# pixeru/bpm_analysis

Hardware: AMD Instinct MI355X
Metric: audio-samples/sec (filter+envelope+peaks), 1024x60s@44.1kHz batch, 1 & 8 GPU (higher is better)
Workload: dtype f64; 1 GPU; 1024 x 60 s 44100 Hz mono int16 recordings per GPU, native mode (filter+envelope+noise floor+raw peaks); mode=native, parallelism=file-sharded x1, batch_pipeline=False

## Files before the change

bpm_analysis_amd/csrc/k_envelope_native.hip:

```cpp
#include <rocfft/rocfft.h>

#include <algorithm>
#include <cstring>
#include <cstdlib>
#include <map>
#include <mutex>
#include <tuple>
#include <vector>

#include <complex>

#include "bpmx_common.h"
#include "bpmx_kernels.h"
#include "bpmx_native.h"
#include "bpmx_hilbert.h"
#ifndef BPMX_NM_POLICY
#define BPMX_NM_POLICY " nt"
#endif
#include "bpmx_qsel.h"
#include "bpmx_xlane.h"

namespace bpmx {

enum { TB_A = 0, TB_V = 0, TB_B = 16, TB_C = 20, TB_D = 24, TB_M = 25, TB_P = 41, TB_ZI = 57, TB_COEF = 64 };

enum { TT_KPOW = 0, TT_MT = 96, TT_G0 = 112, TT_ALPHA = 128, TT_BETA = 384, TT_VI = 640, TT_SIZE = 656 };
constexpr int NAT_PART = 16;
constexpr int NAT_DSMAX = 1280;

struct NatTile {
    int64_t s0;
    int64_t gbase;
    int64_t ybase;
    int32_t j0, nb;
    int32_t f, pad;
};

__device__ __forceinline__ NatTile nat_tile_ld(const NatTile *p, int64_t t) {
    typedef const __attribute__((address_space(4))) int64_t c64;
    c64 *q = (c64 *)(p + __builtin_amdgcn_readfirstlane((int)t));
    NatTile r;
    r.s0 = q[0]; r.gbase = q[1]; r.ybase = q[2];
    const int64_t a = q[3], b = q[4];
    r.j0 = (int32_t)a; r.nb = (int32_t)(a >> 32); r.f = (int32_t)b; r.pad = (int32_t)(b >> 32);
    return r;
}

struct NatBlockArgs {
    const void *pcm;
    const NatTile *tiles;
    int64_t n_tiles, total;
    int32_t bt, channels, ds;
    const double *tab, *tt;
    double *gam;
    double *agg;
    double *part;
};

struct NatCarryArgs {
    const void *pcm;
    const int64_t *foff, *doff, *boff, *toff;
    const int32_t *active;
    int32_t n_files, dtype, channels, ds, bt;
    const double *tab, *tt, *agg;
    double *part;
    double *carry;
    double *yd;
    InitOutArgs io;
    const double *ttab;
};
constexpr int NAT_TT_ROWS = NAT_DSMAX + 20, NAT_TT_PAR = 320;

struct NatYdArgs {
    const NatTile *tiles;
    const int32_t *skip;
    int32_t bt;
    const double *tt, *carry, *gam;
    double *yd;
};

struct NatEnvArgs {
    const double *y;
    const double *h;
    const int64_t *doff;
    const int32_t *active;
    int32_t n_files, window;
    double *env;
    const int32_t *skip;
};

struct V4 { double a, b, c, d; };
struct M4 { double m[16]; };

__device__ __forceinline__ V4 mv(const M4 &M, const V4 &x) {
    V4 r;
    r.a = __builtin_fma(M.m[0], x.a, __builtin_fma(M.m[1], x.b, __builtin_fma(M.m[2], x.c, M.m[3] * x.d)));
    r.b = __builtin_fma(M.m[4], x.a, __builtin_fma(M.m[5], x.b, __builtin_fma(M.m[6], x.c, M.m[7] * x.d)));
    r.c = __builtin_fma(M.m[8], x.a, __builtin_fma(M.m[9], x.b, __builtin_fma(M.m[10], x.c, M.m[11] * x.d)));
    r.d = __builtin_fma(M.m[12], x.a, __builtin_fma(M.m[13], x.b, __builtin_fma(M.m[14], x.c, M.m[15] * x.d)));
    return r;
}
__device__ __forceinline__ V4 mv_rot(const double *r, const V4 &x) {
    const double a1 = r[0], b1 = r[1], a2 = r[2], b2 = r[3];
    return V4{__builtin_fma(a1, x.a, b1 * x.b), __builtin_fma(a1, x.b, -b1 * x.a), __builtin_fma(a2, x.c, b2 * x.d),
              __builtin_fma(a2, x.d, -b2 * x.c)};
}
__device__ __forceinline__ V4 add4(const V4 &x, const V4 &y) { return V4{x.a + y.a, x.b + y.b, x.c + y.c, x.d + y.d}; }
__device__ __forceinline__ V4 acc_rot(const V4 &acc, const double *r, const V4 &x) {
    const double a1 = r[0], b1 = r[1], a2 = r[2], b2 = r[3];
    return V4{__builtin_fma(a1, x.a, __builtin_fma(b1, x.b, acc.a)), __builtin_fma(a1, x.b, __builtin_fma(-b1, x.a, acc.b)),
              __builtin_fma(a2, x.c, __builtin_fma(b2, x.d, acc.c)), __builtin_fma(a2, x.d, __builtin_fma(-b2, x.c, acc.d))};
}
__device__ __forceinline__ M4 mm(const M4 &X, const M4 &Y) {
    M4 R;
#pragma unroll
    for (int i = 0; i < 4; ++i)
#pragma unroll
        for (int j = 0; j < 4; ++j)
            R.m[i * 4 + j] = __builtin_fma(X.m[i * 4 + 0], Y.m[0 * 4 + j],
                             __builtin_fma(X.m[i * 4 + 1], Y.m[1 * 4 + j],
                             __builtin_fma(X.m[i * 4 + 2], Y.m[2 * 4 + j], X.m[i * 4 + 3] * Y.m[3 * 4 + j])));
    return R;
}
__device__ __forceinline__ M4 eye4() {
    M4 R;
#pragma unroll
    for (int i = 0; i < 16; ++i) R.m[i] = (i % 5 == 0) ? 1.0 : 0.0;
    return R;
}
__device__ __forceinline__ M4 shfl_up_m(const M4 &X, int d) {
    M4 R;
#pragma unroll
    for (int i = 0; i < 16; ++i) R.m[i] = __shfl_up(X.m[i], d);
    return R;
}
__device__ __forceinline__ M4 shfl_down_m(const M4 &X, int d) {
    M4 R;
#pragma unroll
    for (int i = 0; i < 16; ++i) R.m[i] = __shfl_down(X.m[i], d);
    return R;
}
__device__ __forceinline__ V4 shfl_v(const V4 &x, int src) {
    return V4{__shfl(x.a, src), __shfl(x.b, src), __shfl(x.c, src), __shfl(x.d, src)};
}
__device__ __forceinline__ V4 shfl_up_v(const V4 &x, int d) {
    return V4{__shfl_up(x.a, d), __shfl_up(x.b, d), __shfl_up(x.c, d), __shfl_up(x.d, d)};
}
__device__ __forceinline__ V4 shfl_down_v(const V4 &x, int d) {
    return V4{__shfl_down(x.a, d), __shfl_down(x.b, d), __shfl_down(x.c, d), __shfl_down(x.d, d)};
}
template <int D>
__device__ __forceinline__ V4 xl_up_v(const V4 &x) {
    return V4{xl_up<D>(x.a), xl_up<D>(x.b), xl_up<D>(x.c), xl_up<D>(x.d)};
}
template <int D>
__device__ __forceinline__ V4 xl_down_v(const V4 &x) {
    return V4{xl_down<D>(x.a), xl_down<D>(x.b), xl_down<D>(x.c), xl_down<D>(x.d)};
}
__device__ __forceinline__ M4 mpow(const M4 &X, int64_t e) {
    M4 R = eye4(), P = X;
    while (e > 0) {
        if (e & 1) R = mm(P, R);
        P = mm(P, P);
        e >>= 1;
    }
    return R;
}

struct SosStep {
    double s[12];
    __device__ __forceinline__ double step(V4 &z, double u) const {
        const double x1 = s[0] * u + z.a;
        const double z00 = s[1] * u - s[4] * x1 + z.b;
        const double z01 = s[2] * u - s[5] * x1;
        const double y = s[6] * x1 + z.c;
        const double z10 = s[7] * x1 - s[10] * y + z.d;
        const double z11 = s[8] * x1 - s[11] * y;
        z = V4{z00, z01, z10, z11};
        return y;
    }
};


template <int DT, bool MULTI>
__device__ __forceinline__ double nat_frame(const void *__restrict__ pcm, int ch, int64_t frame) {
    if (!MULTI) {
        switch (DT) {
        case BPMX_DT_U8: return (double)((const uint8_t *)pcm)[frame];
        case BPMX_DT_I16: return (double)((const int16_t *)pcm)[frame];
        case BPMX_DT_I32: return (double)((const int32_t *)pcm)[frame];
        case BPMX_DT_F32: return (double)((const float *)pcm)[frame];
        default: return ((const double *)pcm)[frame];
        }
    }
    return frame_value(pcm, DT, ch, frame);
}

__device__ __forceinline__ V4 nat_ld4(const double *p) { return V4{p[0], p[1], p[2], p[3]}; }
__device__ __forceinline__ M4 nat_ld16(const double *p) {
    M4 r;
#pragma unroll
    for (int i = 0; i < 16; ++i) r.m[i] = p[i];
    return r;
}
__device__ __forceinline__ double dot4(const V4 &a, const V4 &b) {
    return __builtin_fma(a.a, b.a, __builtin_fma(a.b, b.b, __builtin_fma(a.c, b.c, a.d * b.d)));
}

enum { ET_KPOW = 0, ET_P = 24, ET_C = 40, ET_D = 44, ET_SIZE = 45 };
__device__ __forceinline__ void nat_stage_epilogue_tables(const NatBlockArgs &A, double *et) {
    for (int i = threadIdx.x; i < ET_SIZE; i += blockDim.x) {
        double v;
        if (i < ET_P) v = A.tt[TT_KPOW + i];
        else if (i < ET_C) v = A.tab[TB_P + i - ET_P];
        else if (i < ET_D) v = A.tab[TB_C + i - ET_C];
        else v = A.tab[TB_D];
        et[i] = v;
    }
}

__device__ __forceinline__ void nat_tile_epilogue(const NatBlockArgs &A, const double *et, const NatTile &tl,
                                                  int64_t t, int lane, bool valid, V4 u, V4 v, double x) {
    const int bt = A.bt;
    const int Lt = tl.nb - tl.j0 < bt ? tl.nb - tl.j0 : bt;
    if (Lt < bt) {
        if (valid) {
            double *pp = A.part + ((int64_t)tl.f * 64 + lane) * NAT_PART;
            pp[0] = u.a; pp[1] = u.b; pp[2] = u.c; pp[3] = u.d;
            pp[4] = v.a; pp[5] = v.b; pp[6] = v.c; pp[7] = v.d;
            pp[8] = x;
        }
        return;
    }
    if (!valid) { u = V4{0, 0, 0, 0}; v = V4{0, 0, 0, 0}; x = 0; }
    V4 incl = u;
#define NAT_UP(K)                                                            \
    {                                                                        \
        const V4 y = K == 0 ? xl_up_v<1>(incl) : shfl_up_v(incl, 1 << K);   \
        if (lane >= (1 << K)) incl = acc_rot(incl, et + ET_KPOW + 4 * K, y);   \
    }
    NAT_UP(0) NAT_UP(1) NAT_UP(2) NAT_UP(3) NAT_UP(4) NAT_UP(5)
#undef NAT_UP
    V4 loc = xl_up_v<1>(incl);
    if (lane == 0) loc = V4{0, 0, 0, 0};
    V4 R = valid ? add4(mv(nat_ld16(et + ET_P), loc), v) : V4{0, 0, 0, 0};
#define NAT_DOWN(K)                                                          \
    {                                                                        \
        const V4 y = K == 0 ? xl_down_v<1>(R) : shfl_down_v(R, 1 << K);      \
        if (lane + (1 << K) < 64) R = acc_rot(R, et + ET_KPOW + 4 * K, y);     \
    }
    NAT_DOWN(0) NAT_DOWN(1) NAT_DOWN(2) NAT_DOWN(3) NAT_DOWN(4) NAT_DOWN(5)
#undef NAT_DOWN
    const V4 C = nat_ld4(et + ET_C);
    const double D = et[ET_D];
    if (valid) A.gam[tl.gbase + lane] = dot4(C, R) + D * dot4(C, loc) + D * D * x;
    double *ag = A.agg + t * 8;
    if (lane == bt - 1) { ag[0] = incl.a; ag[1] = incl.b; ag[2] = incl.c; ag[3] = incl.d; }
    if (lane == 0) { ag[4] = R.a; ag[5] = R.b; ag[6] = R.c; ag[7] = R.d; }
}

constexpr int NB_RCH = 20;

__device__ __forceinline__ double nat_lo16(uint32_t w) { return (double)(int)(int16_t)(w & 0xFFFFu); }
__device__ __forceinline__ double nat_hi16(uint32_t w) { return (double)((int)w >> 16); }

typedef uint32_t nat_u4 __attribute__((ext_vector_type(4)));

__global__ __launch_bounds__(64) void k_native_blocks_i16(NatBlockArgs A, const double *__restrict__ coef) {
    typedef nat_u4 u4;
    __shared__ u4 tile[NB_RCH * 64];
    __shared__ double s_et[ET_SIZE];
    nat_stage_epilogue_tables(A, s_et);
    const int lane = threadIdx.x;
    const int16_t *pcm = (const int16_t *)A.pcm;
    const int64_t total = A.total;
    const int ds = A.ds, bt = A.bt;
    const int nch = (7 + bt * ds + 1 + 7) >> 3;
    auto issue = [&](int64_t t, u4 *reg, int &off) {
        const int64_t s0 = nat_tile_ld(A.tiles, t).s0;
        const int64_t a0 = s0 & ~(int64_t)7;
        off = (int)(s0 - a0);
#pragma unroll
        for (int r = 0; r < NB_RCH; ++r) {
            const int q = r * 64 + lane;
            const int64_t c = a0 + (int64_t)q * 8;
            if (q < nch && c + 8 <= total) __builtin_memcpy(&reg[r], pcm + c, 16);
            else reg[r] = u4{0, 0, 0, 0};
        }
    };
    u4 reg[NB_RCH];
    int off = 0;
    int64_t t = blockIdx.x;
    if (t < A.n_tiles) issue(t, reg, off);
    while (t < A.n_tiles) {
        const NatTile tl = nat_tile_ld(A.tiles, t);
#pragma unroll
        for (int r = 0; r < NB_RCH; ++r) tile[r * 64 + lane] = reg[r];
        const int coff = off;
        {
            const int64_t a0 = tl.s0 - coff, tail0 = total & ~(int64_t)7;
            if ((total & 7) && a0 + (int64_t)nch * 8 > tail0 && lane < (int)(total & 7))
                ((int16_t *)tile)[tail0 - a0 + lane] = pcm[tail0 + lane];
        }
        __syncthreads();
        const int64_t tn = t + gridDim.x;
        if (tn < A.n_tiles) issue(tn, reg, off);
        const int j = tl.j0 + lane;
        const bool valid = lane < bt && j < tl.nb;
        double u0 = 0, u1 = 0, u2 = 0, u3 = 0, v0 = 0, v1 = 0, v2 = 0, v3 = 0, x0 = 0;
        if (valid) {
            const int base = coff + lane * ds;
            const uint32_t *wp = (const uint32_t *)tile + (base >> 1);
            const uint32_t sh = (base & 1) ? 16u : 0u;
            auto acc = [&](double xv, const double *c) {
                u0 = __builtin_fma(c[0], xv, u0); u1 = __builtin_fma(c[1], xv, u1);
                u2 = __builtin_fma(c[2], xv, u2); u3 = __builtin_fma(c[3], xv, u3);
                v0 = __builtin_fma(c[4], xv, v0); v1 = __builtin_fma(c[5], xv, v1);
                v2 = __builtin_fma(c[6], xv, v2); v3 = __builtin_fma(c[7], xv, v3);
            };
            const int L = ds + 1;
            int i = 0;
            for (; i + 8 <= L; i += 8) {
                const uint32_t *p = wp + i / 2;
                const uint32_t w0 = p[0], w1 = p[1], w2 = p[2], w3 = p[3], w4 = p[4];
                const uint32_t d0 = __builtin_amdgcn_alignbit(w1, w0, sh);
                const uint32_t d1 = __builtin_amdgcn_alignbit(w2, w1, sh);
                const uint32_t d2 = __builtin_amdgcn_alignbit(w3, w2, sh);
                const uint32_t d3 = __builtin_amdgcn_alignbit(w4, w3, sh);
                const double *cr = coef + (int64_t)i * 8;
                acc(nat_lo16(d0), cr + 0);  acc(nat_hi16(d0), cr + 8);
                acc(nat_lo16(d1), cr + 16); acc(nat_hi16(d1), cr + 24);
                acc(nat_lo16(d2), cr + 32); acc(nat_hi16(d2), cr + 40);
                acc(nat_lo16(d3), cr + 48); acc(nat_hi16(d3), cr + 56);
            }
            const int16_t *th = (const int16_t *)tile;
            for (; i < L; ++i) acc((double)th[base + i], coef + (int64_t)i * 8);
            x0 = (double)th[base];
        }
        nat_tile_epilogue(A, s_et, tl, t, lane, valid, V4{u0, u1, u2, u3}, V4{v0, v1, v2, v3}, x0);
        __syncthreads();
        t = tn;
// ... 18 lines not shown
            const int nvalid = (int)min((int64_t)A.bt, (int64_t)tl.nb - tl.j0);
            const int nfr = nvalid * ds + 1;
            const uint32_t *src = (const uint32_t *)A.pcm + tl.s0;
            for (int k = lane; k < nfr; k += 64) s_fr[k] = src[k];
            __syncthreads();
            if (valid) {
                const double *__restrict__ coef = A.tab + TB_COEF;
                const uint32_t *fr = s_fr + lane * ds;
                for (int i = 0; i <= ds; ++i) {
                    const uint32_t w = fr[i];
                    const double xv = ((double)(int16_t)(w & 0xFFFFu) + (double)(int16_t)(w >> 16)) / 2.0;
                    const double *c = coef + i * 8;
                    u0 = __builtin_fma(c[0], xv, u0); u1 = __builtin_fma(c[1], xv, u1);
                    u2 = __builtin_fma(c[2], xv, u2); u3 = __builtin_fma(c[3], xv, u3);
                    v0 = __builtin_fma(c[4], xv, v0); v1 = __builtin_fma(c[5], xv, v1);
                    v2 = __builtin_fma(c[6], xv, v2); v3 = __builtin_fma(c[7], xv, v3);
                    if (i == 0) x0 = xv;
                }
            }
            nat_tile_epilogue(A, s_et, tl, t, lane, valid, V4{u0, u1, u2, u3}, V4{v0, v1, v2, v3}, x0);
            return;
        }
    }
    if (valid) {
        const double *__restrict__ coef = A.tab + TB_COEF;
        const int64_t fb = tl.s0 + (int64_t)lane * ds;
        for (int i = 0; i <= ds; ++i) {
            const double xv = nat_frame<DT, MULTI>(A.pcm, A.channels, fb + i);
            const double *c = coef + i * 8;
            u0 = __builtin_fma(c[0], xv, u0); u1 = __builtin_fma(c[1], xv, u1);
            u2 = __builtin_fma(c[2], xv, u2); u3 = __builtin_fma(c[3], xv, u3);
            v0 = __builtin_fma(c[4], xv, v0); v1 = __builtin_fma(c[5], xv, v1);
            v2 = __builtin_fma(c[6], xv, v2); v3 = __builtin_fma(c[7], xv, v3);
            if (i == 0) x0 = xv;
        }
    }
    nat_tile_epilogue(A, s_et, tl, t, lane, valid, V4{u0, u1, u2, u3}, V4{v0, v1, v2, v3}, x0);
}

typedef int32_t nm_i4 __attribute__((ext_vector_type(4)));
typedef int32_t nm_i16 __attribute__((ext_vector_type(16)));

constexpr int NM_WAVES = 4;
#ifndef BPMX_NM_SLOTS
#define BPMX_NM_SLOTS 1
#endif
constexpr int NM_SLOTS = BPMX_NM_SLOTS;
constexpr int NM_MINW = 2;
constexpr int NM_NDMA = 18;
constexpr int NM_SLOT_CH = NM_NDMA * 64;

__host__ __device__ constexpr int nm_tile_blocks(int ds, int ks) {
    return ((NM_SLOT_CH * 8 - 7 - 32 * ks - 2) / ds + 1) < 64 ? ((NM_SLOT_CH * 8 - 7 - 32 * ks - 2) / ds + 1) : 64;
}

template <int KS>
__global__ __launch_bounds__(64 * NM_WAVES, NM_MINW) void k_native_blocks_mfma(NatBlockArgs A, const nm_i4 *__restrict__ afrag,
                                                                      const nm_i16 *__restrict__ ainit,
                                                                      const double *__restrict__ cscale) {
    typedef nat_u4 u4;
    __shared__ u4 slots[NM_WAVES * NM_SLOTS][NM_SLOT_CH];
    __shared__ double s_et[ET_SIZE];
    __shared__ nm_i16 s_init[4];
    nat_stage_epilogue_tables(A, s_et);
    for (int i = threadIdx.x; i < 4; i += blockDim.x) s_init[i] = ainit[(i >> 1) * 64 + (i & 1) * 32];
    const int lane = lane_id(), hf = lane >> 5, wv = __builtin_amdgcn_readfirstlane(wave_id());
    const int16_t *pcm = (const int16_t *)A.pcm;
    const int64_t total = A.total;
    const int ds = A.ds, bt = A.bt;
    const int nch = (7 + bt * ds + 1 + 7) >> 3;
    nm_i4 af[2][KS][2];
#pragma unroll
    for (int t = 0; t < 2; ++t)
#pragma unroll
        for (int s = 0; s < KS; ++s)
#pragma unroll
            for (int v = 0; v < 2; ++v) af[t][s][v] = afrag[((t * KS + s) * 2 + v) * 64 + lane];
    double sc[4];
#pragma unroll
    for (int q = 0; q < 4; ++q) sc[q] = cscale[2 * q + hf];
    __syncthreads();

    const int64_t clast = (total & ~(int64_t)7) - 8;
    auto dma = [&](int64_t s0, u4 *slot) {
        const int64_t a0 = s0 & ~(int64_t)7;
        int nchv = nch, lanev = lane;
        asm volatile("" : "+s"(nchv), "+v"(lanev));
#pragma unroll
        for (int r = 0; r < NM_NDMA; ++r) {
            const int q = r * 64 + lanev;
            int64_t c = a0 + (int64_t)q * 8;
            c = (q < nchv && c + 8 <= total) ? c : clast;
            const uint32_t m0 = (uint32_t)(uintptr_t)(__attribute__((address_space(3))) void *)(slot + r * 64);
            asm volatile("s_mov_b32 m0, %1\n\ts_nop 0\n\tglobal_load_lds_dwordx4 %0, off" BPMX_NM_POLICY
                         :: "v"(pcm + c), "s"(m0) : "memory");
        }
    };
    const int64_t stride = (int64_t)gridDim.x * NM_WAVES;
    int64_t t = (int64_t)blockIdx.x * NM_WAVES + wv;
    NatTile tl{};
    if (t < A.n_tiles) tl = nat_tile_ld(A.tiles, t);
    if (t < A.n_tiles) dma(tl.s0, slots[NM_SLOTS * wv]);
    if (NM_SLOTS == 2 && t + stride < A.n_tiles) dma(nat_tile_ld(A.tiles, t + stride).s0, slots[NM_SLOTS * wv + 1]);
    for (int k = 0; t < A.n_tiles; ++k, t += stride) {
        u4 *slot = slots[NM_SLOTS * wv + (NM_SLOTS == 2 ? (k & 1) : 0)];
        const int64_t tr = t + NM_SLOTS * stride;
        NatTile tn{};
        if (tr < A.n_tiles) tn = nat_tile_ld(A.tiles, tr);
        if (NM_SLOTS == 2 && t + stride < A.n_tiles) asm volatile("s_waitcnt vmcnt(%0)" ::"n"(NM_NDMA) : "memory");
        else asm volatile("s_waitcnt vmcnt(0)" ::: "memory");
        __builtin_amdgcn_s_setprio(2);
        const int coff = (int)(tl.s0 & 7);
        {
            const int64_t a0 = tl.s0 - coff, tail0 = total & ~(int64_t)7;
            if ((total & 7) && a0 + (int64_t)nch * 8 > tail0 && lane < (int)(total & 7))
                ((int16_t *)slot)[tail0 - a0 + lane] = pcm[tail0 + lane];
        }
        const int Lt = tl.nb - tl.j0 < bt ? tl.nb - tl.j0 : bt;
        const uint32_t *tw = (const uint32_t *)slot;
        double res[2][4] = {{0, 0, 0, 0}, {0, 0, 0, 0}};
#pragma unroll
        for (int n = 0; n < 2; ++n) {
            const int b = 32 * n + (lane & 31);
            const int hw0 = coff + (b < Lt ? b : 0) * ds + 16 * hf;
            const uint32_t sh = (hw0 & 1) ? 16u : 0u;
            nm_i16 acc0 = s_init[hf], acc1 = s_init[2 + hf];
#ifdef BPMX_NM_NOMFMA
            acc0[0] += (int)tw[hw0 >> 1];
#else
#pragma unroll
            for (int s = 0; s < KS; ++s) {
                const uint32_t *p = tw + ((hw0 + 32 * s) >> 1);
                uint32_t w[9];
#pragma unroll
                for (int i = 0; i < 9; ++i) w[i] = p[i];
                nm_i4 bh, bl;
#pragma unroll
                for (int i = 0; i < 4; ++i) {
                    const uint32_t e0 = __builtin_amdgcn_alignbit(w[2 * i + 1], w[2 * i], sh);
                    const uint32_t e1 = __builtin_amdgcn_alignbit(w[2 * i + 2], w[2 * i + 1], sh);
                    bh[i] = (int32_t)__builtin_amdgcn_perm(e1, e0, 0x07050301u);
                    bl[i] = (int32_t)(__builtin_amdgcn_perm(e1, e0, 0x06040200u) ^ 0x80808080u);
                }
                acc0 = __builtin_amdgcn_mfma_i32_32x32x32_i8(af[0][s][0], bl, acc0, 0, 0, 0);
                acc1 = __builtin_amdgcn_mfma_i32_32x32x32_i8(af[1][s][0], bl, acc1, 0, 0, 0);
                acc0 = __builtin_amdgcn_mfma_i32_32x32x32_i8(af[0][s][1], bh, acc0, 0, 0, 0);
                acc1 = __builtin_amdgcn_mfma_i32_32x32x32_i8(af[1][s][1], bh, acc1, 0, 0, 0);
            }
#endif
#pragma unroll
            for (int q = 0; q < 4; ++q) {
                const int32_t p01 = acc0[4 * q] + acc0[4 * q + 1] * 256, p23 = acc0[4 * q + 2] + acc0[4 * q + 3] * 256;
                const int32_t p45 = acc1[4 * q] + acc1[4 * q + 1] * 256, p67 = acc1[4 * q + 2] + acc1[4 * q + 3] * 256;
                const double L = __builtin_fma((double)p23, 65536.0, (double)p01);
                const double H = __builtin_fma((double)p67, 65536.0, (double)p45);
                res[n][q] = __builtin_fma(H, 4294967296.0, L) * sc[q];
            }
        }
        const int j = tl.j0 + lane;
        const bool valid = lane < bt && j < tl.nb;
        const double x0 = valid ? (double)((const int16_t *)slot)[coff + lane * ds] : 0.0;
        asm volatile("s_waitcnt lgkmcnt(0)" ::: "memory");
        if (tr < A.n_tiles) dma(tn.s0, slot);
        __builtin_amdgcn_s_setprio(0);
        double cf[8];
#pragma unroll
        for (int q = 0; q < 4; ++q) {
            const double other = __shfl_xor(hf ? res[0][q] : res[1][q], 32);
            cf[2 * q] = hf ? other : res[0][q];
            cf[2 * q + 1] = hf ? res[1][q] : other;
// ... 116 lines not shown
                const int hw0 = coff + (b < Ls ? b : 0) * bstride + 16 * g4;
                const uint32_t sh = (hw0 & 1) ? 16u : 0u;
                nm_i4 l[4], h[4];
#pragma unroll
                for (int m = 0; m < 4; ++m) { l[m] = s_init[m][g4]; h[m] = nm_i4{0, 0, 0, 0}; }
#ifndef BPMX_NB_SKIP_MFMA
                const uint32_t *p = tw + (hw0 >> 1);
                uint32_t w[9];
#pragma unroll
                for (int i = 0; i < 9; ++i) w[i] = p[i];
#pragma unroll
                for (int s = 0; s < KS; ++s) {
                    nm_i4 bh, bl;
#pragma unroll
                    for (int i = 0; i < 4; ++i) {
                        const uint32_t e0w = __builtin_amdgcn_alignbit(w[2 * i + 1], w[2 * i], sh);
                        const uint32_t e1w = __builtin_amdgcn_alignbit(w[2 * i + 2], w[2 * i + 1], sh);
                        bh[i] = (int32_t)__builtin_amdgcn_perm(e1w, e0w, 0x07050301u);
                        bl[i] = (int32_t)(__builtin_amdgcn_perm(e1w, e0w, 0x06040200u) ^ 0x80808080u);
                    }
                    if (s + 1 < KS) {
#pragma unroll
                        for (int i = 0; i < 9; ++i) w[i] = p[32 * (s + 1) + i];
                    }
#pragma unroll
                    for (int m = 0; m < 4; ++m) {
                        l[m] = __builtin_amdgcn_mfma_i32_16x16x64_i8(af[m][s], bl, l[m], 0, 0, 0);
                        h[m] = __builtin_amdgcn_mfma_i32_16x16x64_i8(af[m][s], bh, h[m], 0, 0, 0);
                    }
                }
#else
                l[0][0] = (int)tw[hw0 >> 1];
#endif
                double v2[2];
#pragma unroll
                for (int k = 0; k < 2; ++k) {
                    const nm_i4 la = l[2 * k], lb = l[2 * k + 1], ha = h[2 * k], hb = h[2 * k + 1];
                    const double r0 = (double)la[0], r1 = (double)(la[1] + ha[0]);
                    const double r2 = (double)(la[2] + ha[1]), r3 = (double)(la[3] + ha[2]);
                    const double r4 = (double)(lb[0] + ha[3]), r5 = (double)(lb[1] + hb[0]);
                    const double r6 = (double)(lb[2] + hb[1]), r7 = (double)(lb[3] + hb[2]);
                    const double L = __builtin_fma(r3, 16777216.0, __builtin_fma(r2, 65536.0, __builtin_fma(r1, 256.0, r0)));
                    const double H = __builtin_fma(r7, 16777216.0, __builtin_fma(r6, 65536.0, __builtin_fma(r5, 256.0, r4)));
                    v2[k] = __builtin_fma(H, 4294967296.0, L);
                }
                val0 = v2[0] * sc0;
                val1 = v2[1] * sc1;
            }
            const int c = lane - u * bs;
            const bool mine = c >= 0 && c < Ls;
            if (mine) {
                const int16_t *fr = (const int16_t *)slot + coff + c * bstride;
                x0 = ch == 2 ? 0.5 * (double)((int)fr[0] + (int)fr[1]) : (double)fr[0];
            }
            asm volatile("s_waitcnt lgkmcnt(0)" ::: "memory");
            if (pt < A.n_tiles) produce(slot);
            const int src = mine ? c : 0;
#pragma unroll
            for (int q = 0; q < 4; ++q) {
                const double e = __shfl(val0, src + 16 * q), o = __shfl(val1, src + 16 * q);
                if (mine) { cf[2 * q] = e; cf[2 * q + 1] = o; }
            }
        }
        const int j = tl.j0 + lane;
        const bool valid = lane < bt && j < tl.nb;
#ifndef BPMX_NB_SKIP_EPI
        nat_tile_epilogue(A, s_et, tl, t, lane, valid, V4{cf[0], cf[1], cf[2], cf[3]}, V4{cf[4], cf[5], cf[6], cf[7]},
                          x0);
#else
        if (valid && cf[0] == 12345.0) A.gam[0] = x0;
#endif
    }
}
template __global__ void k_native_blocks_mfma_big<5, NB_SLOTS, NB_NDMA, NB_WAVES>(NatBlockArgs, const nm_i4 *, const nm_i4 *,
                                                                                const double *, int);
template __global__ void k_native_blocks_mfma_big<10, NB_SLOTS, NB_NDMA, NB_WAVES>(NatBlockArgs, const nm_i4 *, const nm_i4 *,
                                                                                 const double *, int);

constexpr int ND_WAVES = 4;
constexpr int ND_LDS = 160 * 1024;

inline int nd_ndma(int ds) {
    const int coef = (ds + 1) * 64;
    const int n = (ND_LDS - coef - 1024) / (ND_WAVES * 1024);
    return n < 38 ? n : 38;
}
inline int nd_tile_blocks(int ds, int ch) {
    const int n = nd_ndma(ds);
    if (n < 1) return 0;
    const int b = ((n * 64 * 8 - 7) / ch - 1) / ds;
    return b < 32 ? b : 32;
}
inline size_t nd_lds_bytes(int ds) { return (size_t)nd_ndma(ds) * ND_WAVES * 1024 + (size_t)(ds + 1) * 64 + ET_SIZE * 8; }

template <int CH>
__global__ __launch_bounds__(64 * ND_WAVES, 1) void k_native_blocks_dma(NatBlockArgs A, int ndma) {
    typedef nat_u4 u4;
    extern __shared__ __align__(16) unsigned char nd_smem[];
    const int ds = A.ds, bt = A.bt;
    const int slot_ch = ndma * 64;
    u4 *slots = (u4 *)nd_smem;
    double *s_coef = (double *)(slots + ND_WAVES * slot_ch);
    double *s_et = s_coef + (ds + 1) * 8;
    nat_stage_epilogue_tables(A, s_et);
    {
        const double2 *src = (const double2 *)(A.tab + TB_COEF);
        double2 *dst = (double2 *)s_coef;
        for (int k = threadIdx.x; k < (ds + 1) * 4; k += blockDim.x) dst[k] = src[k];
    }
    const int lane = lane_id(), wv = __builtin_amdgcn_readfirstlane(wave_id());
    const int16_t *pcm = (const int16_t *)A.pcm;
    const int64_t total = A.total;
    const int nch = (7 + (bt * ds + 1) * CH + 7) >> 3;
    __syncthreads();
    const int64_t clast = (total & ~(int64_t)7) - 8;
    auto dma = [&](int64_t e0, u4 *slot) {
        const int64_t a0 = e0 & ~(int64_t)7;
        for (int r = 0; r < ndma; ++r) {
            const int q = r * 64 + lane;
            int64_t c = a0 + (int64_t)q * 8;
            c = (q < nch && c + 8 <= total) ? c : clast;
            const uint32_t m0 = (uint32_t)(uintptr_t)(__attribute__((address_space(3))) void *)(slot + r * 64);
            asm volatile("s_mov_b32 m0, %1\n\ts_nop 0\n\tglobal_load_lds_dwordx4 %0, off"
                         :: "v"(pcm + c), "s"(m0) : "memory");
        }
    };
    const int64_t stride = (int64_t)gridDim.x * ND_WAVES;
    int64_t t = (int64_t)blockIdx.x * ND_WAVES + wv;
    u4 *slot = slots + wv * slot_ch;
    const int blk = lane & 31, hf = lane >> 5;
    const int half = (ds + 2) >> 1;
    const int i0 = hf ? half : 0, i1 = hf ? ds + 1 : half;
    NatTile tl{};
    if (t < A.n_tiles) {
        tl = nat_tile_ld(A.tiles, t);
        dma(tl.s0 * CH, slot);
    }
    for (; t < A.n_tiles; t += stride) {
        const int64_t tr = t + stride;
        NatTile tn{};
        if (tr < A.n_tiles) tn = nat_tile_ld(A.tiles, tr);
        asm volatile("s_waitcnt vmcnt(0)" ::: "memory");
        const int64_t e0 = tl.s0 * CH;
        const int coff = (int)(e0 & 7);
        {
            const int64_t a0 = e0 - coff, tail0 = total & ~(int64_t)7;
            if ((total & 7) && a0 + (int64_t)nch * 8 > tail0 && lane < (int)(total & 7))
                ((int16_t *)slot)[tail0 - a0 + lane] = pcm[tail0 + lane];
            __builtin_amdgcn_wave_barrier();
        }
        const int Lt = tl.nb - tl.j0 < bt ? tl.nb - tl.j0 : bt;
        double u0 = 0, u1 = 0, u2 = 0, u3 = 0, v0 = 0, v1 = 0, v2 = 0, v3 = 0, x0 = 0;
        if (blk < Lt) {
            auto acc = [&](double xv, int i) {
                const double2 *c2 = (const double2 *)(s_coef + i * 8);
                const double2 ca = c2[0], cb = c2[1], cc = c2[2], cd = c2[3];
                u0 = __builtin_fma(ca.x, xv, u0); u1 = __builtin_fma(ca.y, xv, u1);
                u2 = __builtin_fma(cb.x, xv, u2); u3 = __builtin_fma(cb.y, xv, u3);
                v0 = __builtin_fma(cc.x, xv, v0); v1 = __builtin_fma(cc.y, xv, v1);
                v2 = __builtin_fma(cd.x, xv, v2); v3 = __builtin_fma(cd.y, xv, v3);
            };
            if constexpr (CH == 2) {
                const uint32_t *fr = (const uint32_t *)slot + (coff >> 1) + blk * ds;
                auto sum = [](uint32_t w) { return (double)((int)(int16_t)(w & 0xFFFFu) + ((int)w >> 16)); };
                x0 = sum(fr[0]);
                int i = i0;
                for (; i + 4 <= i1; i += 4) {
// ... 584 lines not shown
        for (int c = 0; c < 4; ++c) {
            LD acc = 0;
            for (int k = 0; k < 4; ++k) acc += Cv[k] * V.m[k * 4 + c];
            c2[c] = acc;
        }
        for (int k = 0; k < 4; ++k) { Bv[k] = b2[k]; Cv[k] = c2[k]; }
    } else {
        for (int i = 0; i < 16; ++i) V.m[i] = Vi.m[i] = (i % 5 == 0) ? 1 : 0;
    }
    std::vector<LM> pw(L + 2);
    for (int i = 0; i < 16; ++i) pw[0].m[i] = (i % 5 == 0) ? 1 : 0;
    for (int i = 1; i <= L + 1; ++i) pw[i] = lm_mul(A, pw[i - 1]);
    std::vector<LD> AB((size_t)(L + 1) * 4), h(L + 1);
    for (int i = 0; i <= L; ++i) {
        lm_vec(pw[i], Bv, &AB[(size_t)i * 4]);
        LD acc = 0;
        for (int k = 0; k < 4; ++k) acc += Cv[k] * AB[(size_t)i * 4 + k];
        h[i] = acc;
    }
    LM P;
    for (int i = 0; i < 16; ++i) P.m[i] = 0;
    for (int i = 1; i <= L; ++i) {
        LD CA[4];
        for (int c = 0; c < 4; ++c) {
            LD acc = 0;
            for (int k = 0; k < 4; ++k) acc += Cv[k] * pw[i].m[k * 4 + c];
            CA[c] = acc;
        }
        for (int r = 0; r < 4; ++r)
            for (int c = 0; c < 4; ++c) P.m[r * 4 + c] += AB[(size_t)(i - 1) * 4 + r] * CA[c];
    }
    std::vector<double> out(64 + 8 * (size_t)(L + 1) + TT_SIZE, 0.0);
    for (int i = 0; i < 16; ++i) out[TB_V + i] = (double)V.m[i];
    for (int i = 0; i < 4; ++i) { out[TB_B + i] = (double)Bv[i]; out[TB_C + i] = (double)Cv[i]; }
    out[TB_D] = (double)D;
    for (int i = 0; i < 16; ++i) { out[TB_M + i] = (double)pw[L].m[i]; out[TB_P + i] = (double)P.m[i]; }
    for (int i = 0; i < 4; ++i) out[TB_ZI + i] = sos_zi[i];
    for (int ip = 0; ip <= L; ++ip) {
        double *c = &out[TB_COEF + (size_t)ip * 8];
        if (ip < L) {
            LD F[4];
            lm_vec(pw[L - 1 - ip], Bv, F);
            for (int k = 0; k < 4; ++k) c[k] = (double)F[k];
        }
        LD g[4] = {0, 0, 0, 0};
        if (ip >= 1)
            for (int k = 0; k < 4; ++k) g[k] = AB[(size_t)(ip - 1) * 4 + k] * D;
        for (int i = ip + 1; i <= L; ++i)
            for (int k = 0; k < 4; ++k) g[k] += AB[(size_t)(i - 1) * 4 + k] * h[i - 1 - ip];
        for (int k = 0; k < 4; ++k) c[4 + k] = (double)g[k];
        if (coefld) {
            LD *cl = &(*coefld)[(size_t)ip * 8];
            if (ip < L) lm_vec(pw[L - 1 - ip], Bv, cl);
            else cl[0] = cl[1] = cl[2] = cl[3] = 0;
            for (int k = 0; k < 4; ++k) cl[4 + k] = g[k];
        }
    }
    {
        const LM &M = pw[L];
        std::vector<LM> Mp(T + 1);
        for (int i = 0; i < 16; ++i) Mp[0].m[i] = (i % 5 == 0) ? 1 : 0;
        for (int b = 1; b <= T; ++b) Mp[b] = lm_mul(M, Mp[b - 1]);
        std::vector<LM> G(T + 1);
        for (int i = 0; i < 16; ++i) G[T].m[i] = 0;
        for (int b = T - 1; b >= 0; --b) {
            const LM a = lm_mul(P, Mp[b]), c = lm_mul(M, G[b + 1]);
            for (int i = 0; i < 16; ++i) G[b].m[i] = a.m[i] + c.m[i];
        }
        auto rowC = [&](const LM &X, LD *r) {
            for (int c2 = 0; c2 < 4; ++c2) {
                LD acc = 0;
                for (int k = 0; k < 4; ++k) acc += Cv[k] * X.m[k * 4 + c2];
                r[c2] = acc;
            }
        };
        double *tt = &out[TB_COEF + 8 * (size_t)(L + 1)];
        LM K = M;
        for (int k = 0; k < 6; ++k) {
            tt[TT_KPOW + 4 * k + 0] = (double)K.m[0];
            tt[TT_KPOW + 4 * k + 1] = (double)K.m[1];
            tt[TT_KPOW + 4 * k + 2] = (double)K.m[10];
            tt[TT_KPOW + 4 * k + 3] = (double)K.m[11];
            K = lm_mul(K, K);
        }
        for (int i = 0; i < 16; ++i) tt[TT_VI + i] = (double)Vi.m[i];
        for (int i = 0; i < 16; ++i) { tt[TT_MT + i] = (double)Mp[T].m[i]; tt[TT_G0 + i] = (double)G[0].m[i]; }
        for (int b = 0; b < T; ++b) {
            LD al[4], cg[4], cm[4];
            rowC(Mp[T - b], al);
            rowC(G[b], cg);
            rowC(Mp[b], cm);
            for (int k = 0; k < 4; ++k) {
                tt[TT_ALPHA + 4 * b + k] = (double)al[k];
                tt[TT_BETA + 4 * b + k] = (double)(cg[k] + D * cm[k]);
            }
        }
    }
    return out;
}

constexpr int NM_P = 54, NM_D = 7;
std::vector<int32_t> build_mfma(const std::vector<LD> &cl, int R, int KS) {
    std::vector<int64_t> q((size_t)R * 8);
    std::vector<double> scale(8);
    for (int c = 0; c < 8; ++c) {
        LD mx = 0;
        for (int i = 0; i < R; ++i) mx = std::max(mx, fabsl(cl[(size_t)i * 8 + c]));
        int e = 0;
        if (mx > 0) frexpl(mx, &e);
        scale[c] = ldexp(1.0, e - NM_P);
        for (int i = 0; i < R; ++i) q[(size_t)i * 8 + c] = llroundl(ldexpl(cl[(size_t)i * 8 + c], NM_P - e));
    }
    std::vector<int8_t> d((size_t)R * 64, 0);
    for (int i = 0; i < R * 8; ++i) {
        int64_t v = q[i];
        for (int r = 0; r < NM_D; ++r) {
            int dg = (int)(v & 255);
            if (dg >= 128) dg -= 256;
            d[(size_t)i * 8 + r] = (int8_t)dg;
            v = (v - dg) >> 8;
        }
    }
    auto dig = [&](int k, int c, int r) -> int { return (k < R && r >= 0 && r < 8) ? d[((size_t)k * 8 + c) * 8 + r] : 0; };
    std::vector<int32_t> w(16 + 2 * 64 * 16 + (size_t)2 * KS * 2 * 64 * 4, 0);
    std::memcpy(w.data(), scale.data(), 64);
    int32_t *init = w.data() + 16;
    for (int t = 0; t < 2; ++t)
        for (int l = 0; l < 64; ++l)
            for (int reg = 0; reg < 16; ++reg) {
                const int c = 2 * (reg >> 2) + (l >> 5), r = 4 * t + (reg & 3);
                int64_t sum = 0;
                for (int k = 0; k < R; ++k) sum += dig(k, c, r);
                init[(t * 64 + l) * 16 + reg] = (int32_t)(128 * sum);
            }
    int32_t *af = init + 2 * 64 * 16;
    for (int t = 0; t < 2; ++t)
        for (int st = 0; st < KS; ++st)
            for (int v = 0; v < 2; ++v)
                for (int l = 0; l < 64; ++l) {
                    const int rho = l & 31;
                    const int c = 2 * (rho >> 3) + ((rho >> 2) & 1), r = 4 * t + (rho & 3) - v;
                    for (int j = 0; j < 16; ++j) {
                        const int k = 32 * st + 16 * (l >> 5) + j;
                        const uint32_t byte = (uint8_t)(int8_t)dig(k, c, r);
                        af[(((t * KS + st) * 2 + v) * 64 + l) * 4 + j / 4] |= (int32_t)(byte << (8 * (j & 3)));
                    }
                }
    return w;
}

std::vector<int32_t> build_mfma_big(const std::vector<LD> &cl, int R, int KS, int CH) {
    std::vector<int64_t> q((size_t)R * 8);
    std::vector<double> scale(8);
    for (int c = 0; c < 8; ++c) {
        LD mx = 0;
        for (int i = 0; i < R; ++i) mx = std::max(mx, fabsl(cl[(size_t)i * 8 + c]));
        int e = 0;
        if (mx > 0) frexpl(mx, &e);
        scale[c] = ldexp(1.0, e - NM_P);
        for (int i = 0; i < R; ++i) q[(size_t)i * 8 + c] = llroundl(ldexpl(cl[(size_t)i * 8 + c], NM_P - e));
    }
    std::vector<int8_t> d((size_t)R * 64, 0);
    for (int i = 0; i < R * 8; ++i) {
        int64_t v = q[i];
        for (int r = 0; r < NM_D; ++r) {
            int dg = (int)(v & 255);
// ... 458 lines not shown
```

Before: 1156 billion audio-samples/s.

## Use DPP row-scan with per-lane power tables in native tile epilogue; fast DMA path

Replaces the Kogge-Stone shuffle-based affine scan in the tile epilogue with a DPP row-shift scan. Intra-row steps use kpow tables, and cross-row steps use per-lane precomputed rotation powers (new RPOW table, 32 entries). The backward scan now reverses lanes and reuses the forward scan instead of shfl_down. Separately, the PCM-to-LDS DMA gains a fast path that uses a scalar base address plus lane offset for full chunks when the tile is in bounds. The epilogue constant block grows, so the LDS budget for DMA slots is reduced by 1 KiB, which may lower ndma for some ds.

```diff
diff --git a/bpm_analysis_amd/csrc/bpmx_nat_epilogue.h b/bpm_analysis_amd/csrc/bpmx_nat_epilogue.h
--- /dev/null
+++ b/bpm_analysis_amd/csrc/bpmx_nat_epilogue.h
@@ -0,0 +1,193 @@
+#ifndef BPMX_NAT_EPILOGUE_H
+#define BPMX_NAT_EPILOGUE_H
+
+#include <hip/hip_runtime.h>
+#include <cstdint>
+
+#include "bpmx_xlane.h"
+
+namespace bpmx {
+
+enum { TB_A = 0, TB_V = 0, TB_B = 16, TB_C = 20, TB_D = 24, TB_M = 25, TB_P = 41, TB_ZI = 57, TB_COEF = 64 };
+
+enum { TT_KPOW = 0, TT_MT = 96, TT_G0 = 112, TT_ALPHA = 128, TT_BETA = 384, TT_VI = 640, TT_RPOW = 656, TT_SIZE = 784 };
+constexpr int NAT_PART = 16;
+constexpr int NAT_DSMAX = 1280;
+
+struct NatTile {
+    int64_t s0;
+    int64_t gbase;
+    int64_t ybase;
+    int32_t j0, nb;
+    int32_t f, pad;
+};
+
+struct NatBlockArgs {
+    const void *pcm;
+    const NatTile *tiles;
+    int64_t n_tiles, total;
+    int32_t bt, channels, ds;
+    const double *tab, *tt;
+    double *gam;
+    double *agg;
+    double *part;
+};
+
+struct V4 { double a, b, c, d; };
+struct M4 { double m[16]; };
+
+__device__ __forceinline__ V4 mv(const M4 &M, const V4 &x) {
+    V4 r;
+    r.a = __builtin_fma(M.m[0], x.a, __builtin_fma(M.m[1], x.b, __builtin_fma(M.m[2], x.c, M.m[3] * x.d)));
+    r.b = __builtin_fma(M.m[4], x.a, __builtin_fma(M.m[5], x.b, __builtin_fma(M.m[6], x.c, M.m[7] * x.d)));
+    r.c = __builtin_fma(M.m[8], x.a, __builtin_fma(M.m[9], x.b, __builtin_fma(M.m[10], x.c, M.m[11] * x.d)));
+    r.d = __builtin_fma(M.m[12], x.a, __builtin_fma(M.m[13], x.b, __builtin_fma(M.m[14], x.c, M.m[15] * x.d)));
+    return r;
+}
+__device__ __forceinline__ V4 mv_rot(const double *r, const V4 &x) {
+    const double a1 = r[0], b1 = r[1], a2 = r[2], b2 = r[3];
+    return V4{__builtin_fma(a1, x.a, b1 * x.b), __builtin_fma(a1, x.b, -b1 * x.a), __builtin_fma(a2, x.c, b2 * x.d),
+              __builtin_fma(a2, x.d, -b2 * x.c)};
+}
+__device__ __forceinline__ V4 add4(const V4 &x, const V4 &y) { return V4{x.a + y.a, x.b + y.b, x.c + y.c, x.d + y.d}; }
+__device__ __forceinline__ V4 acc_rot(const V4 &acc, const double *r, const V4 &x) {
+    const double a1 = r[0], b1 = r[1], a2 = r[2], b2 = r[3];
+    return V4{__builtin_fma(a1, x.a, __builtin_fma(b1, x.b, acc.a)), __builtin_fma(a1, x.b, __builtin_fma(-b1, x.a, acc.b)),
+              __builtin_fma(a2, x.c, __builtin_fma(b2, x.d, acc.c)), __builtin_fma(a2, x.d, __builtin_fma(-b2, x.c, acc.d))};
+}
+__device__ __forceinline__ V4 shfl_v(const V4 &x, int src) {
+    return V4{__shfl(x.a, src), __shfl(x.b, src), __shfl(x.c, src), __shfl(x.d, src)};
+}
+__device__ __forceinline__ V4 shfl_up_v(const V4 &x, int d) {
+    return V4{__shfl_up(x.a, d), __shfl_up(x.b, d), __shfl_up(x.c, d), __shfl_up(x.d, d)};
+}
+__device__ __forceinline__ V4 shfl_down_v(const V4 &x, int d) {
+    return V4{__shfl_down(x.a, d), __shfl_down(x.b, d), __shfl_down(x.c, d), __shfl_down(x.d, d)};
+}
+template <int D>
+__device__ __forceinline__ V4 xl_up_v(const V4 &x) {
+    return V4{xl_up<D>(x.a), xl_up<D>(x.b), xl_up<D>(x.c), xl_up<D>(x.d)};
+}
+template <int D>
+__device__ __forceinline__ V4 xl_down_v(const V4 &x) {
+    return V4{xl_down<D>(x.a), xl_down<D>(x.b), xl_down<D>(x.c), xl_down<D>(x.d)};
+}
+__device__ __forceinline__ V4 nat_ld4(const double *p) { return V4{p[0], p[1], p[2], p[3]}; }
+__device__ __forceinline__ M4 nat_ld16(const double *p) {
+    M4 r;
+#pragma unroll
+    for (int i = 0; i < 16; ++i) r.m[i] = p[i];
+    return r;
+}
+__device__ __forceinline__ double dot4(const V4 &a, const V4 &b) {
+    return __builtin_fma(a.a, b.a, __builtin_fma(a.b, b.b, __builtin_fma(a.c, b.c, a.d * b.d)));
+}
+
+enum { ET_KPOW = 0, ET_P = 24, ET_C = 40, ET_D = 44, ET_RPOW = 46, ET_SIZE = ET_RPOW + 128 };
+__device__ __forceinline__ void nat_stage_epilogue_tables(const NatBlockArgs &A, double *et) {
+    for (int i = threadIdx.x; i < ET_SIZE; i += blockDim.x) {
+        double v;
+        if (i < ET_P) v = A.tt[TT_KPOW + i];
+        else if (i < ET_C) v = A.tab[TB_P + i - ET_P];
+        else if (i < ET_D) v = A.tab[TB_C + i - ET_C];
+        else if (i < ET_RPOW) v = A.tab[TB_D];
+        else v = A.tt[TT_RPOW + i - ET_RPOW];
+        et[i] = v;
+    }
+}
+
+template <int CTRL, int ROWS>
+__device__ __forceinline__ double nat_dpp0(double v) {
+    const uint64_t u = (uint64_t)__double_as_longlong(v);
+    const uint32_t lo = (uint32_t)__builtin_amdgcn_update_dpp(0, (int)(uint32_t)u, CTRL, ROWS, 0xf, true);
+    const uint32_t hi = (uint32_t)__builtin_amdgcn_update_dpp(0, (int)(uint32_t)(u >> 32), CTRL, ROWS, 0xf, true);
+    return __longlong_as_double((long long)((uint64_t)lo | ((uint64_t)hi << 32)));
+}
+template <int CTRL, int ROWS>
+__device__ __forceinline__ V4 nat_dpp0_v(const V4 &x) {
+    return V4{nat_dpp0<CTRL, ROWS>(x.a), nat_dpp0<CTRL, ROWS>(x.b), nat_dpp0<CTRL, ROWS>(x.c), nat_dpp0<CTRL, ROWS>(x.d)};
+}
+
+__device__ __forceinline__ V4 nat_row_scan(V4 s, const double *kpow, const double *rpow, int lane) {
+    asm volatile("" : "+v"(lane));
+    double r16[4], r32[4];
+#pragma unroll
+    for (int i = 0; i < 4; ++i) {
+        r16[i] = rpow[4 * (lane & 15) + i];
+        r32[i] = rpow[4 * (lane & 31) + i];
+    }
+    s = acc_rot(s, kpow + 0, nat_dpp0_v<0x111, 0xf>(s));
+    s = acc_rot(s, kpow + 4, nat_dpp0_v<0x112, 0xf>(s));
+    s = acc_rot(s, kpow + 8, nat_dpp0_v<0x114, 0xf>(s));
+    s = acc_rot(s, kpow + 12, nat_dpp0_v<0x118, 0xf>(s));
+    s = acc_rot(s, r16, nat_dpp0_v<0x142, 0xa>(s));
+    s = acc_rot(s, r32, nat_dpp0_v<0x143, 0xc>(s));
+    return s;
+}
+
+#ifdef BPMX_NAT_KS_SCAN
+constexpr bool NAT_KS_SCAN = true;
+#else
+constexpr bool NAT_KS_SCAN = false;
+#endif
+template <bool KS = NAT_KS_SCAN>
+__device__ __forceinline__ void nat_tile_epilogue(const NatBlockArgs &A, const double *et, const NatTile &tl,
+                                                  int64_t t, int lane, bool valid, V4 u, V4 v, double x) {
+    const int bt = A.bt;
+    const int Lt = tl.nb - tl.j0 < bt ? tl.nb - tl.j0 : bt;
+    if (Lt < bt) {
+        if (valid) {
+            double *pp = A.part + ((int64_t)tl.f * 64 + lane) * NAT_PART;
+            pp[0] = u.a; pp[1] = u.b; pp[2] = u.c; pp[3] = u.d;
+            pp[4] = v.a; pp[5] = v.b; pp[6] = v.c; pp[7] = v.d;
+            pp[8] = x;
+        }
+        return;
+    }
+    if (!valid) { u = V4{0, 0, 0, 0}; v = V4{0, 0, 0, 0}; x = 0; }
+    if constexpr (!KS) {
+        const V4 incl = nat_row_scan(u, et + ET_KPOW, et + ET_RPOW, lane);
+        __builtin_amdgcn_sched_barrier(0);
+        V4 loc = xl_up_v<1>(incl);
+        if (lane == 0) loc = V4{0, 0, 0, 0};
+        const V4 w = valid ? add4(mv(nat_ld16(et + ET_P), loc), v) : V4{0, 0, 0, 0};
+        __builtin_amdgcn_sched_barrier(0);
+        const V4 Rr = nat_row_scan(shfl_v(w, 63 - lane), et + ET_KPOW, et + ET_RPOW, lane);
+        const V4 C = nat_ld4(et + ET_C);
+        const double D = et[ET_D];
+        const double cr = __shfl(dot4(C, Rr), 63 - lane);
+        if (valid) A.gam[tl.gbase + lane] = cr + D * dot4(C, loc) + D * D * x;
+        double *ag = A.agg + t * 8;
+        if (lane == bt - 1) { ag[0] = incl.a; ag[1] = incl.b; ag[2] = incl.c; ag[3] = incl.d; }
+        if (lane == 63) { ag[4] = Rr.a; ag[5] = Rr.b; ag[6] = Rr.c; ag[7] = Rr.d; }
+        return;
+    }
+    V4 incl = u;
+#define NAT_UP(K)                                                            \
+    {                                                                        \
+        const V4 y = K == 0 ? xl_up_v<1>(incl) : shfl_up_v(incl, 1 << K);   \
+        if (lane >= (1 << K)) incl = acc_rot(incl, et + ET_KPOW + 4 * K, y);   \
+    }
+    NAT_UP(0) NAT_UP(1) NAT_UP(2) NAT_UP(3) NAT_UP(4) NAT_UP(5)
+#undef NAT_UP
+    V4 loc = xl_up_v<1>(incl);
+    if (lane == 0) loc = V4{0, 0, 0, 0};
+    V4 R = valid ? add4(mv(nat_ld16(et + ET_P), loc), v) : V4{0, 0, 0, 0};
+#define NAT_DOWN(K)                                                          \
+    {                                                                        \
+        const V4 y = K == 0 ? xl_down_v<1>(R) : shfl_down_v(R, 1 << K);      \
+        if (lane + (1 << K) < 64) R = acc_rot(R, et + ET_KPOW + 4 * K, y);     \
+    }
+    NAT_DOWN(0) NAT_DOWN(1) NAT_DOWN(2) NAT_DOWN(3) NAT_DOWN(4) NAT_DOWN(5)
+#undef NAT_DOWN
+    const V4 C = nat_ld4(et + ET_C);
+    const double D = et[ET_D];
+    if (valid) A.gam[tl.gbase + lane] = dot4(C, R) + D * dot4(C, loc) + D * D * x;
+    double *ag = A.agg + t * 8;
+    if (lane == bt - 1) { ag[0] = incl.a; ag[1] = incl.b; ag[2] = incl.c; ag[3] = incl.d; }
+    if (lane == 0) { ag[4] = R.a; ag[5] = R.b; ag[6] = R.c; ag[7] = R.d; }
+}
+
+}
+
+#endif
diff --git a/bpm_analysis_amd/csrc/k_envelope_native.hip b/bpm_analysis_amd/csrc/k_envelope_native.hip
--- a/bpm_analysis_amd/csrc/k_envelope_native.hip
+++ b/bpm_analysis_amd/csrc/k_envelope_native.hip
@@ -19,22 +19,9 @@
 #endif
 #include "bpmx_qsel.h"
 #include "bpmx_xlane.h"
+#include "bpmx_nat_epilogue.h"
 
 namespace bpmx {
-
-enum { TB_A = 0, TB_V = 0, TB_B = 16, TB_C = 20, TB_D = 24, TB_M = 25, TB_P = 41, TB_ZI = 57, TB_COEF = 64 };
-
-enum { TT_KPOW = 0, TT_MT = 96, TT_G0 = 112, TT_ALPHA = 128, TT_BETA = 384, TT_VI = 640, TT_SIZE = 656 };
-constexpr int NAT_PART = 16;
-constexpr int NAT_DSMAX = 1280;
-
-struct NatTile {
-    int64_t s0;
-    int64_t gbase;
-    int64_t ybase;
-    int32_t j0, nb;
-    int32_t f, pad;
-};
 
 __device__ __forceinline__ NatTile nat_tile_ld(const NatTile *p, int64_t t) {
     typedef const __attribute__((address_space(4))) int64_t c64;
@@ -45,17 +32,6 @@
     r.j0 = (int32_t)a; r.nb = (int32_t)(a >> 32); r.f = (int32_t)b; r.pad = (int32_t)(b >> 32);
     return r;
 }
-
-struct NatBlockArgs {
-    const void *pcm;
-    const NatTile *tiles;
-    int64_t n_tiles, total;
-    int32_t bt, channels, ds;
-    const double *tab, *tt;
-    double *gam;
-    double *agg;
-    double *part;
-};
 
 struct NatCarryArgs {
     const void *pcm;
@@ -89,28 +65,6 @@
     const int32_t *skip;
 };
 
-struct V4 { double a, b, c, d; };
-struct M4 { double m[16]; };
-
-__device__ __forceinline__ V4 mv(const M4 &M, const V4 &x) {
-    V4 r;
-    r.a = __builtin_fma(M.m[0], x.a, __builtin_fma(M.m[1], x.b, __builtin_fma(M.m[2], x.c, M.m[3] * x.d)));
-    r.b = __builtin_fma(M.m[4], x.a, __builtin_fma(M.m[5], x.b, __builtin_fma(M.m[6], x.c, M.m[7] * x.d)));
-    r.c = __builtin_fma(M.m[8], x.a, __builtin_fma(M.m[9], x.b, __builtin_fma(M.m[10], x.c, M.m[11] * x.d)));
-    r.d = __builtin_fma(M.m[12], x.a, __builtin_fma(M.m[13], x.b, __builtin_fma(M.m[14], x.c, M.m[15] * x.d)));
-    return r;
-}
-__device__ __forceinline__ V4 mv_rot(const double *r, const V4 &x) {
-    const double a1 = r[0], b1 = r[1], a2 = r[2], b2 = r[3];
-    return V4{__builtin_fma(a1, x.a, b1 * x.b), __builtin_fma(a1, x.b, -b1 * x.a), __builtin_fma(a2, x.c, b2 * x.d),
-              __builtin_fma(a2, x.d, -b2 * x.c)};
-}
-__device__ __forceinline__ V4 add4(const V4 &x, const V4 &y) { return V4{x.a + y.a, x.b + y.b, x.c + y.c, x.d + y.d}; }
-__device__ __forceinline__ V4 acc_rot(const V4 &acc, const double *r, const V4 &x) {
-    const double a1 = r[0], b1 = r[1], a2 = r[2], b2 = r[3];
-    return V4{__builtin_fma(a1, x.a, __builtin_fma(b1, x.b, acc.a)), __builtin_fma(a1, x.b, __builtin_fma(-b1, x.a, acc.b)),
-              __builtin_fma(a2, x.c, __builtin_fma(b2, x.d, acc.c)), __builtin_fma(a2, x.d, __builtin_fma(-b2, x.c, acc.d))};
-}
 __device__ __forceinline__ M4 mm(const M4 &X, const M4 &Y) {
     M4 R;
 #pragma unroll
@@ -139,23 +93,6 @@
 #pragma unroll
     for (int i = 0; i < 16; ++i) R.m[i] = __shfl_down(X.m[i], d);
     return R;
-}
-__device__ __forceinline__ V4 shfl_v(const V4 &x, int src) {
-    return V4{__shfl(x.a, src), __shfl(x.b, src), __shfl(x.c, src), __shfl(x.d, src)};
-}
-__device__ __forceinline__ V4 shfl_up_v(const V4 &x, int d) {
-    return V4{__shfl_up(x.a, d), __shfl_up(x.b, d), __shfl_up(x.c, d), __shfl_up(x.d, d)};
-}
-__device__ __forceinline__ V4 shfl_down_v(const V4 &x, int d) {
-    return V4{__shfl_down(x.a, d), __shfl_down(x.b, d), __shfl_down(x.c, d), __shfl_down(x.d, d)};
-}
-template <int D>
-__device__ __forceinline__ V4 xl_up_v(const V4 &x) {
-    return V4{xl_up<D>(x.a), xl_up<D>(x.b), xl_up<D>(x.c), xl_up<D>(x.d)};
-}
-template <int D>
-__device__ __forceinline__ V4 xl_down_v(const V4 &x) {
-    return V4{xl_down<D>(x.a), xl_down<D>(x.b), xl_down<D>(x.c), xl_down<D>(x.d)};
 }
 __device__ __forceinline__ M4 mpow(const M4 &X, int64_t e) {
     M4 R = eye4(), P = X;
@@ -194,69 +131,6 @@
         }
     }
     return frame_value(pcm, DT, ch, frame);
-}
-
-__device__ __forceinline__ V4 nat_ld4(const double *p) { return V4{p[0], p[1], p[2], p[3]}; }
-__device__ __forceinline__ M4 nat_ld16(const double *p) {
-    M4 r;
-#pragma unroll
-    for (int i = 0; i < 16; ++i) r.m[i] = p[i];
-    return r;
-}
-__device__ __forceinline__ double dot4(const V4 &a, const V4 &b) {
-    return __builtin_fma(a.a, b.a, __builtin_fma(a.b, b.b, __builtin_fma(a.c, b.c, a.d * b.d)));
-}
-
-enum { ET_KPOW = 0, ET_P = 24, ET_C = 40, ET_D = 44, ET_SIZE = 45 };
-__device__ __forceinline__ void nat_stage_epilogue_tables(const NatBlockArgs &A, double *et) {
-    for (int i = threadIdx.x; i < ET_SIZE; i += blockDim.x) {
-        double v;
-        if (i < ET_P) v = A.tt[TT_KPOW + i];
-        else if (i < ET_C) v = A.tab[TB_P + i - ET_P];
-        else if (i < ET_D) v = A.tab[TB_C + i - ET_C];
-        else v = A.tab[TB_D];
-        et[i] = v;
-    }
-}
-
-__device__ __forceinline__ void nat_tile_epilogue(const NatBlockArgs &A, const double *et, const NatTile &tl,
-                                                  int64_t t, int lane, bool valid, V4 u, V4 v, double x) {
-    const int bt = A.bt;
-    const int Lt = tl.nb - tl.j0 < bt ? tl.nb - tl.j0 : bt;
-    if (Lt < bt) {
-        if (valid) {
-            double *pp = A.part + ((int64_t)tl.f * 64 + lane) * NAT_PART;
-            pp[0] = u.a; pp[1] = u.b; pp[2] = u.c; pp[3] = u.d;
-            pp[4] = v.a; pp[5] = v.b; pp[6] = v.c; pp[7] = v.d;
-            pp[8] = x;
-        }
-        return;
-    }
-    if (!valid) { u = V4{0, 0, 0, 0}; v = V4{0, 0, 0, 0}; x = 0; }
-    V4 incl = u;
-#define NAT_UP(K)                                                            \
-    {                                                                        \
-        const V4 y = K == 0 ? xl_up_v<1>(incl) : shfl_up_v(incl, 1 << K);   \
-        if (lane >= (1 << K)) incl = acc_rot(incl, et + ET_KPOW + 4 * K, y);   \
-    }
-    NAT_UP(0) NAT_UP(1) NAT_UP(2) NAT_UP(3) NAT_UP(4) NAT_UP(5)
-#undef NAT_UP
-    V4 loc = xl_up_v<1>(incl);
-    if (lane == 0) loc = V4{0, 0, 0, 0};
-    V4 R = valid ? add4(mv(nat_ld16(et + ET_P), loc), v) : V4{0, 0, 0, 0};
-#define NAT_DOWN(K)                                                          \
-    {                                                                        \
-        const V4 y = K == 0 ? xl_down_v<1>(R) : shfl_down_v(R, 1 << K);      \
-        if (lane + (1 << K) < 64) R = acc_rot(R, et + ET_KPOW + 4 * K, y);     \
-    }
-    NAT_DOWN(0) NAT_DOWN(1) NAT_DOWN(2) NAT_DOWN(3) NAT_DOWN(4) NAT_DOWN(5)
-#undef NAT_DOWN
-    const V4 C = nat_ld4(et + ET_C);
-    const double D = et[ET_D];
-    if (valid) A.gam[tl.gbase + lane] = dot4(C, R) + D * dot4(C, loc) + D * D * x;
-    double *ag = A.agg + t * 8;
-    if (lane == bt - 1) { ag[0] = incl.a; ag[1] = incl.b; ag[2] = incl.c; ag[3] = incl.d; }
-    if (lane == 0) { ag[4] = R.a; ag[5] = R.b; ag[6] = R.c; ag[7] = R.d; }
 }
 
 constexpr int NB_RCH = 20;
@@ -441,10 +315,33 @@
     __syncthreads();
 
     const int64_t clast = (total & ~(int64_t)7) - 8;
+    const uint32_t lane16 = (uint32_t)lane * 16;
     auto dma = [&](int64_t s0, u4 *slot) {
         const int64_t a0 = s0 & ~(int64_t)7;
         int nchv = nch, lanev = lane;
         asm volatile("" : "+s"(nchv), "+v"(lanev));
+#ifndef BPMX_NM_NODMAFAST
+        const uint64_t ga = (uint64_t)(uintptr_t)(pcm + a0);
+        const uint64_t gs = (uint64_t)(uint32_t)__builtin_amdgcn_readfirstlane((int)(uint32_t)ga) |
+                            ((uint64_t)(uint32_t)__builtin_amdgcn_readfirstlane((int)(uint32_t)(ga >> 32)) << 32);
+        if (gs + NM_SLOT_CH * 16 <= (uint64_t)(uintptr_t)(pcm + total)) {
+            const int nfull = nchv >> 6;
+#pragma unroll
+            for (int r = 0; r < NM_NDMA; ++r) {
+                const uint32_t m0 = (uint32_t)(uintptr_t)(__attribute__((address_space(3))) void *)(slot + r * 64);
+                if (r < nfull) {
+                    asm volatile("s_mov_b32 m0, %2\n\ts_nop 0\n\tglobal_load_lds_dwordx4 %0, %1" BPMX_NM_POLICY
+                                 :: "v"(lane16), "s"(gs + r * 1024), "s"(m0) : "memory");
+                } else {
+                    const int q = r * 64 + lanev;
+                    const int64_t c = q < nchv ? a0 + (int64_t)q * 8 : clast;
+                    asm volatile("s_mov_b32 m0, %1\n\ts_nop 0\n\tglobal_load_lds_dwordx4 %0, off" BPMX_NM_POLICY
+                                 :: "v"(pcm + c), "s"(m0) : "memory");
+                }
+            }
+            return;
+        }
+#endif
 #pragma unroll
         for (int r = 0; r < NM_NDMA; ++r) {
             const int q = r * 64 + lanev;
@@ -727,7 +624,8 @@
 
 inline int nd_ndma(int ds) {
     const int coef = (ds + 1) * 64;
-    const int n = (ND_LDS - coef - 1024) / (ND_WAVES * 1024);
+    static_assert(ET_SIZE * 8 <= 2048, "epilogue constants: 2 KiB of the LDS budget");
+    const int n = (ND_LDS - coef - 2048) / (ND_WAVES * 1024);
     return n < 38 ? n : 38;
 }
 inline int nd_tile_blocks(int ds, int ch) {
@@ -1478,6 +1376,12 @@
             tt[TT_KPOW + 4 * k + 2] = (double)K.m[10];
             tt[TT_KPOW + 4 * k + 3] = (double)K.m[11];
             K = lm_mul(K, K);
+        }
+        K = M;
+        for (int d = 1; d <= 32; ++d) {
+            double *r = &tt[TT_RPOW + 4 * (d - 1)];
+            r[0] = (double)K.m[0]; r[1] = (double)K.m[1]; r[2] = (double)K.m[10]; r[3] = (double)K.m[11];
+            K = lm_mul(M, K);
         }
         for (int i = 0; i < 16; ++i) tt[TT_VI + i] = (double)Vi.m[i];
         for (int i = 0; i < 16; ++i) { tt[TT_MT + i] = (double)Mp[T].m[i]; tt[TT_G0 + i] = (double)G[0].m[i]; }
```

Result: faster. 1172 billion audio-samples/s (median of 6 runs) (+1.4%).
